# Refefer/Dampr

Hardware: AMD Instinct MI355X
Metric: tfidf_rows_per_sec (higher is better)
Workload: dtype int64-exact; 1 GPU; model=tfidf-docfreq, corpus_mb_per_gpu=10240, vocab=100000, global_batch=111848106, seq_len=96, parallelism=dp1

## Files before the change

dampr_amd/gpu/tfidf.py:

```python
import os

import torch

from ..ops import native
from .relational import _pow2_at_least

MODE_NEWLINE = 0
MODE_TOKEN_START = 1


def chunk_bounds(text, chunk_bytes):
    n = text.numel()
    bounds = [0]
    while bounds[-1] < n:
        e = min(bounds[-1] + chunk_bytes, n)
        if e < n:
            nl = torch.nonzero(text[e - 1:e + (1 << 16)] == ord("\n"))
            e = e + int(nl[0].item()) if nl.numel() else n
        bounds.append(e)
    return bounds


class TfidfEngine(object):
    def __init__(self, device, vocab_capacity=1 << 21):
        self.ext = native.require()
        self.device = torch.device(device)
        self.cap = _pow2_at_least(vocab_capacity)
        opts = dict(dtype=torch.int64, device=self.device)
        self.cnt_keys = torch.zeros(self.cap, **opts)
        self.cnt_vals = torch.zeros(self.cap, **opts)
        self.dict_keys = torch.zeros(self.cap, **opts)
        self.dict_vals = torch.zeros(self.cap, **opts)
        self.seen = None
        self._fb_seen = None
        self._err = None
        self._ablate = 0
        self.n_docs = 0

    def reset(self):
        self.cnt_keys.zero_()
        self.cnt_vals.zero_()
        self.dict_keys.zero_()
        self.dict_vals.zero_()
        self.n_docs = 0


    def positions(self, text, mode):
        counts = self.ext.mark_counts(text, mode).to(torch.int64)
        offsets = torch.cumsum(counts, 0) - counts
        total = int(offsets[-1].item() + counts[-1].item())
        out = torch.empty(total, dtype=torch.int32, device=self.device)
        self.ext.mark_positions(text, mode, offsets.to(torch.int32), out)
        return out, total


    def count_chunk(self, text, pos_base=0):
        assert text.numel() < (1 << 31), "chunk must be < 2 GiB"
        if self._fb_seen is None:
            self._fb_seen = torch.zeros(1 << 22, dtype=torch.int64,
                                        device=self.device)
            self._err = torch.zeros(4, dtype=torch.int32,
                                    device=self.device)
        else:
            self._fb_seen.zero_()
            self._err.zero_()
        snap = (self.cnt_keys.clone(), self.cnt_vals.clone(),
                self.dict_keys.clone(), self.dict_vals.clone())
        self.ext.tfidf_count_docs(text, self.cnt_keys, self.cnt_vals,
                                  self.dict_keys, self.dict_vals, pos_base,
                                  self._fb_seen, self._err, self._ablate)
        err, _, n_docs, _ = self._err.tolist()
        doc_base = self.n_docs
        self.n_docs += n_docs
        if err:
            (self.cnt_keys, self.cnt_vals,
             self.dict_keys, self.dict_vals) = snap
            nl, _ = self.positions(text, MODE_NEWLINE)
            self._count_chunk_general(text, nl, pos_base, doc_base)
        return n_docs

    def _count_chunk_general(self, text, nl, pos_base, doc_base):
        ts, n_tok = self.positions(text, MODE_TOKEN_START)
        seen_cap = _pow2_at_least(2 * max(n_tok, 1))
        if self.seen is None or self.seen.numel() < seen_cap:
            self.seen = torch.zeros(seen_cap, dtype=torch.int64,
                                    device=self.device)
        else:
            self.seen.zero_()
        self.ext.tfidf_count(text, nl, ts, self.seen, self.cnt_keys,
                             self.cnt_vals, self.dict_keys, self.dict_vals,
                             pos_base, doc_base)


    def extract(self):
        n_out = int((self.cnt_keys != 0).sum().item())
        out_k, out_v, _cur = self.ext.table_extract(
            self.cnt_keys, self.cnt_vals, n_out)
        order = torch.argsort(out_k)
        return out_k[order], out_v[order]


    def idf(self, df, total_docs):
        return self.ext.idf(df, float(total_docs))

    def _token_layout(self, keys):
        packed = self.ext.table_lookup(self.dict_keys, self.dict_vals, keys)
        lens = (packed & 0xFF).to(torch.int64)
        offsets = torch.cumsum(lens, 0) - lens
        total = int((offsets[-1] + lens[-1]).item()) if keys.numel() else 0
        return packed, lens, offsets, total

    def token_strings_dev(self, keys, text):
        packed, lens, offsets, total = self._token_layout(keys)
        blob = self.ext.gather_tokens(text, packed, offsets, total)
        return blob, lens

    def merge_exchanged(self, keys, df, blob, lens):
        self.cnt_keys.zero_()
        self.cnt_vals.zero_()
        self.dict_keys.zero_()
        self.dict_vals.zero_()
        self.ext.table_merge(keys, df, self.cnt_keys, self.cnt_vals)
        offsets = torch.cumsum(lens, 0) - lens
        packed = torch.bitwise_or(torch.bitwise_left_shift(offsets, 8),
                                  lens)
        self.ext.table_put(keys, packed, self.dict_keys, self.dict_vals)

    def token_strings(self, keys, text):
        blob, lens = self.token_strings_dev(keys, text)
        return blob.cpu().numpy(), lens.cpu().numpy()

    def sink_tsv_device(self, path, part_id, keys, df, idf, src_text):
        os.makedirs(path, exist_ok=True)
        packed, lens, tok_off, total_tok = self._token_layout(keys)
        sizes = self.ext.tsv_sizes(lens, df, idf)
        row_off = torch.cumsum(sizes, 0) - sizes
        total = int((row_off[-1] + sizes[-1]).item()) if keys.numel() else 0
        blob = self.ext.gather_tokens(src_text, packed, tok_off, total_tok)
        out = self.ext.tsv_format(blob, tok_off, lens, df, idf, row_off,
                                  total)
        with open(os.path.join(path, "part-{}".format(part_id)), "wb") as fh:
            fh.write(out.cpu().numpy().tobytes())


def run_tfidf(text_np, device="cuda:0", sink_path=None, chunk_bytes=None,
              engine=None):
    dev = torch.device(device)
    if isinstance(text_np, torch.Tensor):
        text = text_np.to(dev)
    else:
        text = torch.from_numpy(text_np).to(dev)
    eng = engine or TfidfEngine(dev)
    eng.reset()
    bounds = chunk_bounds(text, chunk_bytes or text.numel())
    for s, e in zip(bounds, bounds[1:]):
        eng.count_chunk(text[s:e].contiguous(), pos_base=s)
    keys, df = eng.extract()
    idf = eng.idf(df, eng.n_docs)
    blob, lens = eng.token_strings(keys, text)
    if sink_path:
        eng.sink_tsv_device(sink_path, 0, keys, df, idf, text)
    out = {}
    pos = 0
    b = blob.tobytes()
    df_np = df.cpu().numpy()
    idf_np = idf.cpu().numpy()
    for i in range(len(lens)):
        ln = int(lens[i])
        out[b[pos:pos + ln].decode("ascii")] = (int(df_np[i]),
                                                float(idf_np[i]))
        pos += ln
    return out
```

dampr_amd/ops/hip/dampr_kernels.hip:

```cpp
#include <hip/hip_runtime.h>
#include "host.h"

#include "common.h"

#define BLOCK 256
#define VBYTES 16
#define TILE (BLOCK * VBYTES)

#define MODE_NEWLINE 0
#define MODE_TOKEN_START 1

__device__ __forceinline__ bool mark_at(int mode, const u8* text,
                                        long i, long n) {
    u8 c = text[i];
    if (mode == MODE_NEWLINE) return c == '\n';
    if (!is_word(c)) return false;
    return i == 0 || !is_word(text[i - 1]);
}

__device__ __forceinline__ u32 nlmask32(u32 w) {
    u32 x = w ^ 0x0A0A0A0Au;
    return (x - 0x01010101u) & ~x & 0x80808080u;
}

__global__ void count_marks_kernel(const u8* __restrict__ text, long n,
                                   int mode, int iters,
                                   u32* __restrict__ counts) {
    long base = (long)blockIdx.x * iters * TILE;
    int tid = threadIdx.x;
    u32 local = 0;
    for (int it = 0; it < iters; ++it) {
        long off = base + (long)it * TILE + (long)tid * VBYTES;
        if (off >= n) break;
        if (off + VBYTES <= n) {
            uint4 v = *reinterpret_cast<const uint4*>(text + off);
            if (mode == MODE_NEWLINE) {
                local += __popc(nlmask32(v.x)) + __popc(nlmask32(v.y))
                       + __popc(nlmask32(v.z)) + __popc(nlmask32(v.w));
            } else {
                const u8* b = reinterpret_cast<const u8*>(&v);
                #pragma unroll
                for (int j = 0; j < VBYTES; ++j) {
                    bool prev_word = (j > 0)
                        ? is_word(b[j - 1])
                        : (off > 0 ? is_word(text[off - 1]) : false);
                    local += is_word(b[j]) && !prev_word;
                }
            }
        } else {
            for (long i = off; i < n; ++i)
                local += mark_at(mode, text, i, n);
        }
    }
    __shared__ u32 wsum[BLOCK / WAVE];
    for (int d = WAVE / 2; d > 0; d >>= 1)
        local += __shfl_down(local, d, WAVE);
    int lane = tid & (WAVE - 1), wid = tid / WAVE;
    if (lane == 0) wsum[wid] = local;
    __syncthreads();
    if (tid == 0) {
        u32 total = 0;
        for (int w = 0; w < BLOCK / WAVE; ++w) total += wsum[w];
        counts[blockIdx.x] = total;
    }
}

#define SCAN_MAX_ITERS 16

__device__ __forceinline__ u32 gather_marks(const u8* __restrict__ text,
                                            long n, int mode, long off,
                                            u8* rel) {
    u32 cnt = 0;
    if (off >= n) return 0;
    if (off + VBYTES <= n) {
        uint4 v = *reinterpret_cast<const uint4*>(text + off);
        if (mode == MODE_NEWLINE) {
            const u32 words[4] = {v.x, v.y, v.z, v.w};
            #pragma unroll
            for (int wi = 0; wi < 4; ++wi) {
                u32 m = nlmask32(words[wi]);
                while (m) {
                    int bit = __ffs(m) - 1;
                    rel[cnt++] = (u8)(wi * 4 + (bit >> 3));
                    m &= m - 1;
                }
            }
            return cnt;
        }
        const u8* b = reinterpret_cast<const u8*>(&v);
        #pragma unroll
        for (int j = 0; j < VBYTES; ++j) {
            u8 c = b[j];
            bool prev_word = (j > 0)
                ? is_word(b[j - 1])
                : (off > 0 ? is_word(text[off - 1]) : false);
            bool m = is_word(c) && !prev_word;
            if (m) rel[cnt++] = (u8)j;
        }
    } else {
        long lim = n - off;
        for (long j = 0; j < lim; ++j)
            if (mark_at(mode, text, off + j, n)) rel[cnt++] = (u8)j;
    }
    return cnt;
}

__global__ void write_marks_kernel(const u8* __restrict__ text, long n,
                                   int mode, int iters,
                                   const u32* __restrict__ block_offsets,
                                   u32* __restrict__ out) {
    long base = (long)blockIdx.x * iters * TILE;
    int tid = threadIdx.x;
    int lane = tid & (WAVE - 1), wid = tid / WAVE;
    __shared__ u32 wtile[BLOCK / WAVE][SCAN_MAX_ITERS];

    for (int it = 0; it < iters; ++it) {
        long off = base + (long)it * TILE + (long)tid * VBYTES;
        u8 rel[VBYTES];
        u32 cnt = gather_marks(text, n, mode, off, rel);
        u32 tot = cnt;
        for (int d = WAVE / 2; d > 0; d >>= 1)
            tot += __shfl_down(tot, d, WAVE);
        if (lane == 0) wtile[wid][it] = tot;
    }
    __syncthreads();

    u32 run = block_offsets[blockIdx.x];
    for (int it = 0; it < iters; ++it) {
        u32 wb = run;
        u32 tile_tot = 0;
        for (int w = 0; w < BLOCK / WAVE; ++w) {
            if (w < wid) wb += wtile[w][it];
            tile_tot += wtile[w][it];
        }
        long off = base + (long)it * TILE + (long)tid * VBYTES;
        u8 rel[VBYTES];
        u32 cnt = gather_marks(text, n, mode, off, rel);
        u32 scan = cnt;
        for (int d = 1; d < WAVE; d <<= 1) {
            u32 x = __shfl_up(scan, d, WAVE);
            if (lane >= d) scan += x;
        }
        u32 excl = wb + scan - cnt;
        for (u32 j = 0; j < cnt; ++j)
            out[excl + j] = (u32)(off + rel[j]);
        run += tile_tot;
    }
}

__global__ void tfidf_count_kernel(
        const u8* __restrict__ text, long n,
        const u32* __restrict__ nl_pos, long n_nl,
        const u32* __restrict__ tok_start, long n_tok,
        u64* __restrict__ seen_keys, u64 seen_mask,
        u64* __restrict__ cnt_keys, u64* __restrict__ cnt_vals,
        u64 cnt_mask,
        u64* __restrict__ dict_keys, u64* __restrict__ dict_vals,
        u64 dict_mask, u64 pos_base, u64 doc_base) {
    long stride = (long)gridDim.x * blockDim.x;
    for (long t = (long)blockIdx.x * blockDim.x + threadIdx.x; t < n_tok;
         t += stride) {
        u32 start = tok_start[t];
        long p = start;
        u64 h = 0;
        u32 j = 0;
        while (p < n) {
            u8 c = text[p];
            if (!is_word(c)) break;
            h = tokmix_step(h, j, lower_ascii(c));
            ++p;
            ++j;
        }
        u32 len = (u32)(p - start);
        h = tokmix_final(h, len);
        long lo = 0, hi = n_nl;
        while (lo < hi) {
            long mid = (lo + hi) >> 1;
            if (nl_pos[mid] < start) lo = mid + 1; else hi = mid;
        }
        u64 doc = (u64)lo + doc_base;
        u64 tok_key = h ? h : 1ULL;
        u64 sk = splitmix64(h ^ (doc * 0x9E3779B97F4A7C15ULL));
        if (!sk) sk = 1;
        u64 slot;
        if (table_insert_u64(seen_keys, seen_mask, sk, &slot)) {
            table_add_u64(cnt_keys, cnt_vals, cnt_mask, tok_key, 1ULL);
            if (table_insert_u64(dict_keys, dict_mask, tok_key, &slot))
                dict_vals[slot] = ((pos_base + (u64)start) << 8)
                                  | (u64)min(len, 255u);
        }
    }
}

#ifndef DOC_WAVES
#define DOC_WAVES 4
#endif
#ifndef STAGE_B
#define STAGE_B 2048
#endif
#define SEG_OVERLAP 272
#ifndef DOC_SET
#define DOC_SET 256
#endif
#ifndef FB_PROBE_CAP
#define FB_PROBE_CAP 512
#endif
#ifndef DOC_SPAN
#define DOC_SPAN 8192
#endif
#ifndef GROUP_BYTES
#define GROUP_BYTES 1024
#endif
#ifndef CCACHE
#define CCACHE 1024
#endif
#ifndef DOC_BPL
#define DOC_BPL 8
#endif
#define DOC_LENMIX_N 128
#define DOC_SALT_K 0x9E3779B97F4A7C15ULL
#define DOC_WIN (WAVE * DOC_BPL)
static_assert(DOC_BPL == 4 || DOC_BPL == 8, "lane word is b32 or b64");
static_assert(STAGE_B % 16 == 0, "stage edge on a lane boundary");
static_assert(DOC_SPAN % 16 == 0 && DOC_SPAN >= 16, "span on a 16 B edge");
static_assert(GROUP_BYTES == WAVE * 16 && GROUP_BYTES <= STAGE_B,
              "group search is one uint4 per lane of staged text");
#define GROUP_OPEN (1L << 62)

__device__ __forceinline__ u32 swar_ge(u32 x7, u32 k) {
    return x7 + (0x80u - k) * 0x01010101u;
}
__device__ __forceinline__ u32 swar_pack4(u32 m) {
    return (((m & 0x80808080u) >> 7) * 0x01020408u) >> 24;
}
__device__ __forceinline__ u32 wordbits4(u32 x) {
    const u32 x7 = x & 0x7F7F7F7Fu;
    const u32 y7 = x7 | 0x20202020u;
    const u32 m = (swar_ge(y7, 'a') ^ swar_ge(y7, 'z' + 1))
                | (swar_ge(x7, '0') ^ swar_ge(x7, '9' + 1))
                | (swar_ge(x7, '_') ^ swar_ge(x7, '_' + 1));
    return swar_pack4(m & ~x);
}
__device__ __forceinline__ u32 nlbits4(u32 x) {
    const u32 v = x ^ 0x0A0A0A0Au;
    return swar_pack4(~(((v & 0x7F7F7F7Fu) + 0x7F7F7F7Fu) | v));
}
__device__ __forceinline__ u32 nlbits16(const u8* p, long at, long from,
                                        long to) {
    const uint4 v = *reinterpret_cast<const uint4*>(p);
    const u32 m = nlbits4(v.x) | (nlbits4(v.y) << 4) | (nlbits4(v.z) << 8)
                | (nlbits4(v.w) << 12);
    const int lo = (int)min(max(from - at, 0L), 16L);
    const int hi = (int)min(max(to - at, 0L), 16L);
    return m & ((1u << hi) - 1u) & ~((1u << lo) - 1u);
}
__device__ __forceinline__ u32 nlbits_from(long at, long pos) {
    const int k = (int)min(max(pos - at, 0L), 16L);
    return ~((1u << k) - 1u);
}
__device__ __forceinline__ u64 low_bytes_mask(int k) {
    return k >= 8 ? ~0ULL : ((1ULL << (8 * k)) - 1ULL);
}

#define CC_PROBES 4
#define CC_HIT 0
#define CC_NEW 1
#define CC_MISS 2
#define EMIT_CNT 1u
#define EMIT_DICT 2u

__device__ __forceinline__ int block_cache_step(
        u64* __restrict__ cck, u32* __restrict__ ccv, u32 slot, u64 key,
        u64 cur) {
    if (cur == key) { atomicAdd(&ccv[slot], 1u); return CC_HIT; }
    if (cur == 0ULL) {
        const u64 prev = atomicCAS(&cck[slot], 0ULL, key);
        if (prev == 0ULL || prev == key) {
            atomicAdd(&ccv[slot], 1u);
            return prev == 0ULL ? CC_NEW : CC_HIT;
        }
    }
    return -1;
}

__device__ __forceinline__ int block_cache_add(
        u64* __restrict__ cck, u32* __restrict__ ccv, u64 key) {
    const u32 s0 = (u32)(key & (CCACHE - 1));
    u64 c[CC_PROBES];
    #pragma unroll
    for (int p = 0; p < CC_PROBES; ++p)
        c[p] = cck[(s0 + p) & (CCACHE - 1)];
    #pragma unroll
    for (int p = 0; p < CC_PROBES; ++p)
        asm volatile("" : "+v"(c[p]));
    int f = CC_PROBES;
    u64 cf = 0;
    #pragma unroll
    for (int p = CC_PROBES - 1; p >= 0; --p)
        if (c[p] == key || c[p] == 0ULL) { f = p; cf = c[p]; }
    if (f == CC_PROBES) return CC_MISS;
    u32 slot = (s0 + f) & (CCACHE - 1);
    int r = block_cache_step(cck, ccv, slot, key, cf);
    if (r >= 0) return r;
    for (int p = f + 1; p < CC_PROBES; ++p) {
        slot = (slot + 1) & (CCACHE - 1);
        r = block_cache_step(cck, ccv, slot, key, cck[slot]);
        if (r >= 0) return r;
    }
    return CC_MISS;
}

__device__ __forceinline__ int lds_set_insert(u64* set, u64 h) {
    u32 slot = (u32)(h & (DOC_SET - 1));
    for (int probe = 0; probe < DOC_SET; ++probe) {
        u64 prev = atomicCAS(&set[slot], 0ULL, h);
        if (prev == 0ULL) return 1;
        if (prev == h) return 0;
        slot = (slot + 1) & (DOC_SET - 1);
    }
    return -1;
}

__global__ void __launch_bounds__(DOC_WAVES * WAVE, 5)
tfidf_docs_kernel(const u8* __restrict__ text, long n,
                  u64* __restrict__ cnt_keys, u64* __restrict__ cnt_vals,
                  u64 cnt_mask,
                  u64* __restrict__ dict_keys, u64* __restrict__ dict_vals,
                  u64 dict_mask, u64 pos_base,
                  u64* __restrict__ fb_seen, u64 fb_mask,
                  u32* __restrict__ err_flag, u32 ablate) {
    __shared__ __align__(16) u8 stage[DOC_WAVES][STAGE_B + 16];
    __shared__ u64 dset[DOC_WAVES][DOC_SET];
    __shared__ u64 cck[CCACHE];
    __shared__ u32 ccv[CCACHE];
    __shared__ u64 toktab[256];
    __shared__ u64 lenmix[DOC_LENMIX_N];
    __shared__ u32 blk_docs;
    static_assert(sizeof(stage) + sizeof(dset) + sizeof(cck) + sizeof(ccv)
                  + sizeof(toktab) + sizeof(lenmix) + 8 <= 32768,
                  "block LDS allows 5 blocks per CU");
    const int wid = __builtin_amdgcn_readfirstlane(threadIdx.x / WAVE);
    const int lane = threadIdx.x % WAVE;
    const long gwave = (long)blockIdx.x * DOC_WAVES + wid;
    const long nwaves = (long)gridDim.x * DOC_WAVES;
    const long nspans = (n + DOC_SPAN - 1) / DOC_SPAN;
    u8* st = stage[wid];
    u64* set = dset[wid];
    u32 my_docs = 0;

    for (int i = threadIdx.x; i < CCACHE; i += blockDim.x) {
        cck[i] = 0;
        ccv[i] = 0;
    }
    for (int i = threadIdx.x; i < 256; i += blockDim.x)
        toktab[i] = is_word((u8)i) ? toktab_entry(lower_ascii((u8)i)) : 0ULL;
    for (int i = threadIdx.x; i < DOC_LENMIX_N; i += blockDim.x)
        lenmix[i] = splitmix64((u64)i);
    if (threadIdx.x == 0) blk_docs = 0;
    __syncthreads();

    auto finish_emit = [&](u64 key, u64 pk, u64 cw, u64 dw, u32 fl) {
        if ((fl & EMIT_DICT) && dw != key) {
            u64 slot;
            if (table_insert_u64(dict_keys, dict_mask, key, &slot))
                dict_vals[slot] = pk;
        }
        if (fl & EMIT_CNT) {
            if (cw == key) atomicAdd(&cnt_vals[key & cnt_mask], 1ULL);
            else table_add_u64(cnt_keys, cnt_vals, cnt_mask, key, 1ULL);
        }
    };

    for (long sp = gwave; sp < nspans; sp += nwaves) {
        const long a = sp * DOC_SPAN;
        const long b = a + DOC_SPAN;
        long win_lo = -1, win_hi = -1, aseg = 0;

        auto stage_at = [&](long seg) {
            aseg = seg & ~15L;
            const int stage_bytes =
                (int)min((long)(STAGE_B + 16), n - aseg);
            if (aseg + STAGE_B + 16 <= n) {
                #pragma unroll
                for (int i = 0; i < STAGE_B; i += WAVE * 16)
                    __builtin_amdgcn_global_load_lds(
                        (const u32*)(text + aseg + i + lane * 16),
                        (u32*)(st + i), 16, 0, 0);
                if (lane == 0)
                    __builtin_amdgcn_global_load_lds(
                        (const u32*)(text + aseg + STAGE_B),
                        (u32*)(st + STAGE_B), 16, 0, 0);
            } else {
                for (int i = lane * 16; i < stage_bytes; i += WAVE * 16) {
                    if (aseg + i + 16 <= n) {
                        *reinterpret_cast<uint4*>(st + i) =
                            *reinterpret_cast<const uint4*>(
                                text + aseg + i);
                    } else {
                        for (int j = i; j < stage_bytes; ++j)
                            st[j] = (aseg + j < n)
                                ? text[aseg + j] : (u8)0;
                    }
                }
            }
            __builtin_amdgcn_s_waitcnt(0x0070);
            asm volatile("" ::: "memory");
            __builtin_amdgcn_wave_barrier();
            win_lo = seg;
            win_hi = aseg + stage_bytes;
        };
        auto nl_lane16 = [&](long base, long from, long to) -> u32 {
            const long at = base + lane * 16;
            return at < to
                ? nlbits16(st + (int)(at - aseg), at, from, to) : 0u;
        };
        auto first_nl = [&](long from, long to) -> long {
            for (long base = from & ~15L; base < to; base += WAVE * 16) {
                const u32 m = nl_lane16(base, from, to);
                const u64 any = __ballot(m != 0);
                if (any) {
                    const int fl = __ffsll((unsigned long long)any) - 1;
                    const u32 mf = __builtin_amdgcn_readlane(m, fl);
                    return base + fl * 16 + (__ffs(mf) - 1);
                }
            }
            return -1;
        };

        long gs = 0;
        if (a > 0) {
            const long lim = min(b - 1, n);
            long p = -1;
            for (long pos = a - 1; pos < lim; ) {
                if (pos < win_lo || pos >= win_hi) stage_at(pos);
                const long to = min(win_hi, lim);
                p = first_nl(pos, to);
                if (p >= 0) break;
                pos = to;
            }
            if (p < 0) continue;
            gs = p + 1;
        }

        while (gs < n) {
            if (gs < win_lo || gs >= win_hi) stage_at(gs);
            const long gbase = gs & ~15L;
            long gend = GROUP_OPEN;
            for (int attempt = 0; attempt < 2; ++attempt) {
                const long to = min(gbase + (long)GROUP_BYTES, win_hi);
                const u32 m = nl_lane16(gbase, gs, to);
                const u32 mh = m & nlbits_from(gbase + lane * 16, b - 1);
                const u64 any = __ballot(m != 0);
                const u64 anyh = __ballot(mh != 0);
                if (anyh) {
                    const int fl = __ffsll((unsigned long long)anyh) - 1;
                    const u32 mf = __builtin_amdgcn_readlane(mh, fl);
                    gend = gbase + fl * 16 + (__ffs(mf) - 1);
                    break;
                }
                long last = -1;
                if (any) {
                    const int ll = 63 - __clzll((long long)any);
                    const u32 ml = __builtin_amdgcn_readlane(m, ll);
                    last = gbase + ll * 16 + (31 - __clz((int)ml));
                }
                if (to == n) {
                    gend = (last == n - 1) ? last : n;
                    break;
                }
                if (last >= 0) { gend = last; break; }
                if (to == gbase + (long)GROUP_BYTES) break;
                stage_at(gs);
            }

            for (int s = lane; s < DOC_SET; s += WAVE) set[s] = 0;
            u32 carry_word = 0;
            u32 carry_len = 0;
            u64 carry_g = 0;
            long carry_start = gs;
            u32 carry_lines = 0;

            auto emit_token = [&](u64 gh, u32 tl, long tbase, int trel,
                                  u32 drel) {
                if (ablate & 1) {
                    if (gh == 0xdeadbeefdeadbeefULL) err_flag[1] = 1;
                    return;
                }
                u64 lm;
                if (tl < DOC_LENMIX_N) lm = lenmix[tl];
                else lm = splitmix64((u64)tl);
                const u64 hh = gh ^ lm;
                const u64 key = hh ? hh : 1ULL;
                const long doc_id = gs + (long)drel;
                u64 dk = hh ^ ((u64)doc_id * DOC_SALT_K);
                if (!dk) dk = 1;
                int fresh = lds_set_insert(set, dk);
                if (fresh < 0) {
                    u64 sk = splitmix64(hh ^ ((u64)doc_id
                                              * 0x9E3779B97F4A7C15ULL));
                    if (!sk) sk = 1;
                    u64 slot = sk & fb_mask;
                    fresh = 0;
                    int probe = 0;
                    while (true) {
                        u64 prev = atomicCAS(&fb_seen[slot], 0ULL, sk);
                        if (prev == 0ULL) { fresh = 1; break; }
                        if (prev == sk) break;
                        slot = (slot + 1) & fb_mask;
                        if (++probe > FB_PROBE_CAP) {
                            atomicOr(err_flag, 1u);
                            break;
                        }
                    }
                }
                u32 fl = 0;
                if (fresh == 1 && !(ablate & 2)) {
                    const int cc = block_cache_add(cck, ccv, key);
                    if (cc == CC_MISS) fl |= EMIT_CNT;
                    if (!(ablate & 4) && cc != CC_HIT) fl |= EMIT_DICT;
                }
                const u64 pk = ((pos_base + (u64)(tbase + trel)) << 8)
                             | (u64)min(tl, 255u);
                u64 cw = 0, dw = 0;
                if (fl & EMIT_CNT) cw = cnt_keys[key & cnt_mask];
                if (fl & EMIT_DICT) dw = dict_keys[key & dict_mask];
                if (fl) finish_emit(key, pk, cw, dw, fl);
            };

            for (long seg = gs; seg < gend; ) {
                if (seg < win_lo || seg >= win_hi) stage_at(seg);
                if (gend == GROUP_OPEN) {
                    const long p = first_nl(seg, win_hi);
                    if (p >= 0) gend = p;
                    else if (win_hi == n) gend = n;
                }
                const long seg_end = min(gend, win_hi);
                const int soff = (int)(seg - aseg);
                const int soff_end = (int)(seg_end - aseg);
                const bool group_continues = seg_end < gend;
                for (int wb = soff & ~(DOC_BPL - 1); wb < soff_end;
                     wb += DOC_WIN) {
                    const int o = wb + lane * DOC_BPL;
                    const int keep_lo = min(max(soff - o, 0), DOC_BPL);
                    const int keep_hi = min(max(soff_end - o, 0), DOC_BPL);
                    u64 raw = 0;
                    if (keep_hi > 0) {
#if DOC_BPL == 8
                        raw = *reinterpret_cast<const u64*>(st + o);
#else
                        raw = *reinterpret_cast<const u32*>(st + o);
#endif
                    }
                    raw &= low_bytes_mask(keep_hi) & ~low_bytes_mask(keep_lo);
                    u32 W = wordbits4((u32)raw);
                    u32 NLb = nlbits4((u32)raw);
#if DOC_BPL == 8
                    W |= wordbits4((u32)(raw >> 32)) << 4;
                    NLb |= nlbits4((u32)(raw >> 32)) << 4;
#endif
                    u64 P[DOC_BPL];
                    u64 acc = 0, pz = 0;
                    u64 T[DOC_BPL];
                    #pragma unroll
                    for (int j = 0; j < DOC_BPL; ++j)
                        T[j] = toktab[(u32)(raw >> (8 * j)) & 0xFFu];
                    #pragma unroll
                    for (int j = 0; j < DOC_BPL; ++j)
                        asm volatile("" : "+v"(T[j]));
                    #pragma unroll
                    for (int j = 0; j < DOC_BPL; ++j) {
                        acc ^= rotl64(T[j], (u32)j);
                        pz = ((W >> j) & 1u) ? pz : acc;
                        P[j] = acc;
                    }
                    const bool first_w = W & 1u;
                    const bool last_w = (W >> (DOC_BPL - 1)) & 1u;
                    const u64 fw = __ballot(first_w);
                    const u64 lw = __ballot(last_w);
                    if (carry_word && !(fw & 1ULL)) {
                        if (lane == 0)
                            emit_token(carry_g, carry_len, carry_start,
                                       0, carry_lines);
                        carry_word = 0;
                        carry_len = 0;
                        carry_g = 0;
                    }
                    const int span = soff_end - wb;
                    const int e = span >= DOC_WIN ? WAVE - 1
                                                  : (span - 1) / DOC_BPL;
                    const bool hold = (e == WAVE - 1) || group_continues;
                    u64 nf = fw;
                    if (hold && e < WAVE - 1) nf |= 1ULL << (e + 1);
                    const bool next_first = (lane == WAVE - 1)
                        ? true : (bool)((nf >> (lane + 1)) & 1ULL);
                    const bool cont_in = first_w
                        && (lane == 0 ? carry_word != 0
                                      : (bool)((lw >> (lane - 1)) & 1ULL));
                    u32 E = W & ~((W >> 1)
                                  | ((u32)next_first << (DOC_BPL - 1)));

                    const u32 zb = ~W & ((1u << DOC_BPL) - 1u);
                    const int ts = zb ? 32 - __clz(zb) : 0;
                    u64 tg = 0;
                    u32 tlen = 0;
                    bool closed = true;
                    if (last_w) {
                        tg = rotl64(acc ^ pz, (u32)(64 - ts));
                        tlen = (u32)(DOC_BPL - ts);
                        closed = !(ts == 0 && cont_in);
                    }
                    for (int d = 1; d < WAVE; d <<= 1) {
                        if (!__ballot(!closed && lane >= d)) break;
                        const u64 ag = __shfl_up(tg, d, WAVE);
                        const u32 al = __shfl_up(tlen, d, WAVE);
                        const int ac = __shfl_up((int)closed, d, WAVE);
                        if (!closed && lane >= d) {
                            tg = ag ^ rotl64(tg, al);
                            tlen += al;
                            closed = ac;
                        }
                    }
                    if (!closed) {
                        tg = carry_g ^ rotl64(tg, carry_len);
                        tlen += carry_len;
                    }
                    u64 pg = __shfl_up(tg, 1, WAVE);
                    u32 plen = __shfl_up(tlen, 1, WAVE);
                    if (lane == 0) { pg = carry_g; plen = carry_len; }

                    const u32 nlc = __popc(NLb);
                    u32 nl_before = carry_lines;
                    for (u32 k = 1; ; ++k) {
                        const u64 b = __ballot(nlc >= k);
                        if (!b) break;
                        nl_before = __builtin_amdgcn_mbcnt_hi(
                            (u32)(b >> 32),
                            __builtin_amdgcn_mbcnt_lo((u32)b, nl_before));
                        carry_lines += (u32)__popcll(b);
                    }

                    if (((lw >> e) & 1ULL) && hold) {
                        carry_word = 1;
                        carry_g = __shfl(tg, e, WAVE);
                        carry_len = (u32)__shfl((int)tlen, e, WAVE);
                        carry_start = aseg + wb + (long)(e + 1) * DOC_BPL
                                      - (long)carry_len;
                    } else {
                        carry_word = 0;
                        carry_len = 0;
                        carry_g = 0;
                    }

                    u64 pprev = 0;
                    while (__ballot(E != 0)) {
                        if (E) {
                            const int j = __ffs(E) - 1;
                            E &= E - 1;
                            u64 pj = P[0];
                            #pragma unroll
                            for (int i = 1; i < DOC_BPL; ++i)
                                pj = (j == i) ? P[i] : pj;
                            const u32 zj = zb & ((1u << j) - 1u);
                            const int s = zj ? 32 - __clz(zj) : 0;
                            u64 g = rotl64(pj ^ pprev, (u32)(64 - s));
                            pprev = pj;
                            u32 len = (u32)(j - s + 1);
                            if (s == 0 && cont_in) {
                                g = pg ^ rotl64(g, plen);
                                len += plen;
                            }
                            emit_token(g, len, aseg,
                                       o + j + 1 - (int)len,
                                       nl_before
                                       + __popc(NLb & ((1u << j) - 1u)));
                        }
                    }
                }
                __builtin_amdgcn_wave_barrier();
                seg = seg_end;
            }
            if (carry_word) {
                if (lane == 0)
                    emit_token(carry_g, carry_len, carry_start, 0,
                               carry_lines);
            }
            my_docs += carry_lines + 1;
            if (gend >= b - 1) break;
            gs = gend + 1;
        }
    }
    if (lane == 0 && my_docs) atomicAdd(&blk_docs, my_docs);

    __syncthreads();
    if (threadIdx.x == 0 && blk_docs) atomicAdd(&err_flag[2], blk_docs);
    for (int i = threadIdx.x; i < CCACHE; i += blockDim.x)
        if (cck[i])
            table_add_u64(cnt_keys, cnt_vals, cnt_mask, cck[i],
                          (u64)ccv[i]);
}

__global__ void table_merge_kernel(const u64* __restrict__ in_keys,
                                   const long* __restrict__ in_vals,
                                   long n, u64* __restrict__ keys,
                                   u64* __restrict__ vals, u64 mask) {
    long stride = (long)gridDim.x * blockDim.x;
    for (long i = (long)blockIdx.x * blockDim.x + threadIdx.x; i < n;
         i += stride) {
        u64 k = in_keys[i];
        if (k) table_add_u64(keys, vals, mask, k, (u64)in_vals[i]);
    }
}

__global__ void table_put_kernel(const u64* __restrict__ in_keys,
                                 const u64* __restrict__ in_vals, long n,
                                 u64* __restrict__ keys,
                                 u64* __restrict__ vals, u64 mask) {
    long stride = (long)gridDim.x * blockDim.x;
    for (long i = (long)blockIdx.x * blockDim.x + threadIdx.x; i < n;
         i += stride) {
        u64 k = in_keys[i];
        if (!k) continue;
        u64 slot;
        if (table_insert_u64(keys, mask, k, &slot))
            vals[slot] = in_vals[i];
    }
}

__global__ void table_extract_kernel(const u64* __restrict__ keys,
                                     const u64* __restrict__ vals,
                                     long cap, u64* __restrict__ out_k,
                                     long* __restrict__ out_v,
                                     u64* __restrict__ cursor) {
    long stride = (long)gridDim.x * blockDim.x;
    for (long i = (long)blockIdx.x * blockDim.x + threadIdx.x; i < cap;
         i += stride) {
        u64 k = keys[i];
        if (k) {
            u64 j = atomicAdd(cursor, 1ULL);
            out_k[j] = k;
            out_v[j] = (long)vals[i];
        }
    }
}

__global__ void table_lookup_kernel(const u64* __restrict__ keys,
                                    const u64* __restrict__ vals, u64 mask,
                                    const u64* __restrict__ query, long n,
                                    u64* __restrict__ out) {
    long stride = (long)gridDim.x * blockDim.x;
    for (long i = (long)blockIdx.x * blockDim.x + threadIdx.x; i < n;
         i += stride) {
        u64 k = query[i];
        u64 slot = k & mask;
        u64 r = 0;
        while (true) {
            u64 cur = keys[slot];
            if (cur == k) { r = vals[slot]; break; }
            if (cur == 0) break;
            slot = (slot + 1) & mask;
        }
        out[i] = r;
    }
}

__global__ void idf_kernel(const long* __restrict__ df, long n,
                           double total, double* __restrict__ out) {
    long stride = (long)gridDim.x * blockDim.x;
    for (long i = (long)blockIdx.x * blockDim.x + threadIdx.x; i < n;
         i += stride)
        out[i] = log(1.0 + total / (double)df[i]);
}

__global__ void gather_tokens_kernel(const u8* __restrict__ text,
                                     const u64* __restrict__ packed, long n,
                                     const long* __restrict__ offsets,
                                     u8* __restrict__ out) {
    long stride = (long)gridDim.x * blockDim.x;
    for (long i = (long)blockIdx.x * blockDim.x + threadIdx.x; i < n;
         i += stride) {
        u64 pk = packed[i];
        u32 pos = (u32)(pk >> 8);
        u32 len = (u32)(pk & 0xFF);
        long o = offsets[i];
        for (u32 j = 0; j < len; ++j)
            out[o + j] = lower_ascii(text[pos + j]);
    }
}


__device__ __forceinline__ int dec_digits_u64(u64 v) {
    int d = 1;
    while (v >= 10) { v /= 10; ++d; }
    return d;
}

__device__ __forceinline__ void fmt_idf_parts(double x, u64* int_part,
                                              u64* frac_part) {
    double scaled = x * 1e9 + 0.5;
    u64 v = (u64)scaled;
    *int_part = v / 1000000000ULL;
    *frac_part = v % 1000000000ULL;
}

__global__ void tsv_sizes_kernel(const long* __restrict__ lens,
                                 const long* __restrict__ df,
                                 const double* __restrict__ idf, long n,
                                 long* __restrict__ sizes) {
    long stride = (long)gridDim.x * blockDim.x;
    for (long i = (long)blockIdx.x * blockDim.x + threadIdx.x; i < n;
         i += stride) {
        u64 ip, fp;
        fmt_idf_parts(idf[i], &ip, &fp);
        sizes[i] = lens[i] + 1 + dec_digits_u64((u64)df[i]) + 1
                 + dec_digits_u64(ip) + 1 + 9 + 1;
    }
}

__device__ __forceinline__ u8* write_u64_dec(u8* p, u64 v, int width) {
    for (int j = width - 1; j >= 0; --j) { p[j] = '0' + (v % 10); v /= 10; }
    return p + width;
}

__global__ void tsv_format_kernel(const u8* __restrict__ blob,
                                  const long* __restrict__ tok_off,
                                  const long* __restrict__ lens,
                                  const long* __restrict__ df,
                                  const double* __restrict__ idf,
                                  const long* __restrict__ row_off, long n,
                                  u8* __restrict__ out) {
    long stride = (long)gridDim.x * blockDim.x;
    for (long i = (long)blockIdx.x * blockDim.x + threadIdx.x; i < n;
         i += stride) {
        u8* p = out + row_off[i];
        const u8* t = blob + tok_off[i];
        for (long j = 0; j < lens[i]; ++j) *p++ = t[j];
        *p++ = '\t';
        u64 d = (u64)df[i];
        p = write_u64_dec(p, d, dec_digits_u64(d));
        *p++ = '\t';
        u64 ip, fp;
        fmt_idf_parts(idf[i], &ip, &fp);
        p = write_u64_dec(p, ip, dec_digits_u64(ip));
        *p++ = '.';
        p = write_u64_dec(p, fp, 9);
        *p++ = '\n';
    }
}


namespace {

inline int grid_for(long work, int block = BLOCK, int cap = 4096) {
    long g = (work + block - 1) / block;
    return (int)std::min<long>(std::max<long>(g, 1), cap);
}

void check_u8(const torch::Tensor& t) {
    TORCH_CHECK(t.is_cuda() && t.dtype() == torch::kUInt8 &&
                t.is_contiguous(), "expected contiguous u8 device tensor");
}

constexpr int SCAN_ITERS = 8;

}

torch::Tensor mark_counts(torch::Tensor text, long mode) {
    check_u8(text);
    long n = text.numel();
    long span = (long)SCAN_ITERS * TILE;
    long nblocks = (n + span - 1) / span;
    auto counts = torch::empty({std::max(nblocks, 1L)},
        torch::TensorOptions().dtype(torch::kUInt32).device(text.device()));
    if (n == 0) { counts.zero_(); return counts; }
    hipLaunchKernelGGL(count_marks_kernel, dim3((u32)nblocks), dim3(BLOCK),
                       0, cur_stream(), text.data_ptr<u8>(), n, (int)mode,
                       SCAN_ITERS, (u32*)counts.data_ptr());
    return counts;
}

void mark_positions(torch::Tensor text, long mode,
                    torch::Tensor block_offsets, torch::Tensor out) {
    check_u8(text);
    long n = text.numel();
    if (n == 0 || out.numel() == 0) return;
    long span = (long)SCAN_ITERS * TILE;
    long nblocks = (n + span - 1) / span;
    hipLaunchKernelGGL(write_marks_kernel, dim3((u32)nblocks), dim3(BLOCK),
                       0, cur_stream(), text.data_ptr<u8>(), n, (int)mode,
                       SCAN_ITERS, (u32*)block_offsets.data_ptr(),
                       (u32*)out.data_ptr());
}

void tfidf_count(torch::Tensor text, torch::Tensor nl_pos,
                 torch::Tensor tok_start, torch::Tensor seen_keys,
                 torch::Tensor cnt_keys, torch::Tensor cnt_vals,
                 torch::Tensor dict_keys, torch::Tensor dict_vals,
                 long pos_base, long doc_base) {
    check_u8(text);
    long n_tok = tok_start.numel();
    if (n_tok == 0) return;
    hipLaunchKernelGGL(tfidf_count_kernel,
        dim3(grid_for(n_tok)), dim3(BLOCK), 0, cur_stream(),
        text.data_ptr<u8>(), text.numel(),
        (const u32*)nl_pos.data_ptr(), nl_pos.numel(),
        (const u32*)tok_start.data_ptr(), n_tok,
        (u64*)seen_keys.data_ptr(), (u64)(seen_keys.numel() - 1),
        (u64*)cnt_keys.data_ptr(), (u64*)cnt_vals.data_ptr(),
        (u64)(cnt_keys.numel() - 1),
        (u64*)dict_keys.data_ptr(), (u64*)dict_vals.data_ptr(),
        (u64)(dict_keys.numel() - 1), (u64)pos_base, (u64)doc_base);
}

void tfidf_count_docs(torch::Tensor text, torch::Tensor cnt_keys,
                      torch::Tensor cnt_vals, torch::Tensor dict_keys,
                      torch::Tensor dict_vals, long pos_base,
                      torch::Tensor fb_seen, torch::Tensor meta,
                      long ablate) {
    check_u8(text);
    TORCH_CHECK(meta.is_cuda() && meta.is_contiguous()
                && meta.scalar_type() == torch::kInt32
                && meta.numel() >= 3, "meta must be device int32[>=3]");
    TORCH_CHECK(text.numel() < (1L << 31), "chunk must be < 2 GiB");
    const long n = text.numel();
    if (n == 0) return;
    long waves_needed = (n + DOC_SPAN - 1) / DOC_SPAN;
    long blocks = std::min<long>((waves_needed + DOC_WAVES - 1) / DOC_WAVES,
                                 8192);
    hipLaunchKernelGGL(tfidf_docs_kernel, dim3((u32)blocks),
        dim3(DOC_WAVES * WAVE), 0, cur_stream(),
        text.data_ptr<u8>(), n,
        (u64*)cnt_keys.data_ptr(), (u64*)cnt_vals.data_ptr(),
        (u64)(cnt_keys.numel() - 1),
        (u64*)dict_keys.data_ptr(), (u64*)dict_vals.data_ptr(),
        (u64)(dict_keys.numel() - 1), (u64)pos_base,
        (u64*)fb_seen.data_ptr(), (u64)(fb_seen.numel() - 1),
        (u32*)meta.data_ptr(), (u32)ablate);
}

long tfidf_span_bytes() { return DOC_SPAN; }

void table_merge(torch::Tensor in_keys, torch::Tensor in_vals,
                 torch::Tensor keys, torch::Tensor vals) {
    long n = in_keys.numel();
    if (n == 0) return;
    hipLaunchKernelGGL(table_merge_kernel, dim3(grid_for(n)), dim3(BLOCK),
        0, cur_stream(), (const u64*)in_keys.data_ptr(),
        in_vals.data_ptr<long>(), n, (u64*)keys.data_ptr(),
        (u64*)vals.data_ptr(), (u64)(keys.numel() - 1));
}

void table_put(torch::Tensor in_keys, torch::Tensor in_vals,
               torch::Tensor keys, torch::Tensor vals) {
    long n = in_keys.numel();
    if (n == 0) return;
    hipLaunchKernelGGL(table_put_kernel, dim3(grid_for(n)), dim3(BLOCK),
        0, cur_stream(), (const u64*)in_keys.data_ptr(),
        (const u64*)in_vals.data_ptr(), n, (u64*)keys.data_ptr(),
        (u64*)vals.data_ptr(), (u64)(keys.numel() - 1));
}

std::vector<torch::Tensor> table_extract(torch::Tensor keys,
                                         torch::Tensor vals, long n_out) {
    auto dev = keys.device();
    auto out_k = torch::empty({n_out},
        torch::TensorOptions().dtype(torch::kInt64).device(dev));
    auto out_v = torch::empty({n_out},
        torch::TensorOptions().dtype(torch::kInt64).device(dev));
    auto cursor = torch::zeros({1},
        torch::TensorOptions().dtype(torch::kInt64).device(dev));
    long cap = keys.numel();
    if (cap > 0 && n_out > 0)
        hipLaunchKernelGGL(table_extract_kernel, dim3(grid_for(cap)),
            dim3(BLOCK), 0, cur_stream(), (const u64*)keys.data_ptr(),
            (const u64*)vals.data_ptr(), cap, (u64*)out_k.data_ptr(),
            out_v.data_ptr<long>(), (u64*)cursor.data_ptr());
    return {out_k, out_v, cursor};
}

torch::Tensor table_lookup(torch::Tensor keys, torch::Tensor vals,
                           torch::Tensor query) {
    long n = query.numel();
    auto out = torch::zeros({n},
        torch::TensorOptions().dtype(torch::kInt64).device(query.device()));
    if (n > 0)
        hipLaunchKernelGGL(table_lookup_kernel, dim3(grid_for(n)),
            dim3(BLOCK), 0, cur_stream(), (const u64*)keys.data_ptr(),
            (const u64*)vals.data_ptr(), (u64)(keys.numel() - 1),
            (const u64*)query.data_ptr(), n, (u64*)out.data_ptr());
    return out;
}

torch::Tensor idf(torch::Tensor df, double total) {
    long n = df.numel();
    auto out = torch::empty({n},
        torch::TensorOptions().dtype(torch::kFloat64).device(df.device()));
    if (n > 0)
        hipLaunchKernelGGL(idf_kernel, dim3(grid_for(n)), dim3(BLOCK), 0,
            cur_stream(), df.data_ptr<long>(), n, total,
            out.data_ptr<double>());
    return out;
}

torch::Tensor gather_tokens(torch::Tensor text, torch::Tensor packed,
                            torch::Tensor offsets, long total_bytes) {
    check_u8(text);
    long n = packed.numel();
    auto out = torch::empty({std::max(total_bytes, 1L)},
        torch::TensorOptions().dtype(torch::kUInt8).device(text.device()));
    if (n > 0)
        hipLaunchKernelGGL(gather_tokens_kernel, dim3(grid_for(n)),
            dim3(BLOCK), 0, cur_stream(), text.data_ptr<u8>(),
            (const u64*)packed.data_ptr(), n, offsets.data_ptr<long>(),
            out.data_ptr<u8>());
    return out;
}

torch::Tensor tsv_sizes(torch::Tensor lens, torch::Tensor df,
                        torch::Tensor idf) {
    long n = lens.numel();
    auto out = torch::empty({std::max(n, 1L)},
        torch::TensorOptions().dtype(torch::kInt64).device(lens.device()));
    if (n > 0)
        hipLaunchKernelGGL(tsv_sizes_kernel, dim3(grid_for(n)), dim3(BLOCK),
            0, cur_stream(), lens.data_ptr<long>(), df.data_ptr<long>(),
            idf.data_ptr<double>(), n, out.data_ptr<long>());
    return out;
}

torch::Tensor tsv_format(torch::Tensor blob, torch::Tensor tok_off,
                         torch::Tensor lens, torch::Tensor df,
                         torch::Tensor idf, torch::Tensor row_off,
                         long total_bytes) {
    long n = lens.numel();
    auto out = torch::empty({std::max(total_bytes, 1L)},
        torch::TensorOptions().dtype(torch::kUInt8).device(blob.device()));
    if (n > 0)
        hipLaunchKernelGGL(tsv_format_kernel, dim3(grid_for(n)),
            dim3(BLOCK), 0, cur_stream(), blob.data_ptr<u8>(),
            tok_off.data_ptr<long>(), lens.data_ptr<long>(),
            df.data_ptr<long>(), idf.data_ptr<double>(),
            row_off.data_ptr<long>(), n, out.data_ptr<u8>());
    return out;
}

torch::Tensor rs_hist(torch::Tensor keys, long shift, long nblocks);
torch::Tensor rs_digit_fold(torch::Tensor keys);
void rs_scatter(torch::Tensor keys, torch::Tensor payload,
                torch::Tensor scanned, long shift, long nblocks,
                torch::Tensor out_k, torch::Tensor out_p);
void seg_reduce(torch::Tensor seg, torch::Tensor vals, torch::Tensor out,
                long op);
void hj_build(torch::Tensor keys_r, torch::Tensor t_keys,
              torch::Tensor t_head, torch::Tensor next);
torch::Tensor hj_count(torch::Tensor keys_l, torch::Tensor t_keys,
                       torch::Tensor t_head, torch::Tensor next,
                       long left_outer);
long rs_span();
torch::Tensor seg_count(torch::Tensor keys);
void seg_reduce_fused(torch::Tensor keys, torch::Tensor vals,
                      torch::Tensor tile_base, long op,
                      torch::Tensor out_keys, torch::Tensor out_vals);
void mp_merge(torch::Tensor ka, torch::Tensor pa, torch::Tensor kb,
              torch::Tensor pb, long bias_signed, torch::Tensor out_k,
              torch::Tensor out_p);
void varlen_gather(torch::Tensor blob, torch::Tensor src_off,
                   torch::Tensor lens, torch::Tensor new_offs,
                   torch::Tensor out);
std::vector<torch::Tensor> hj_emit(torch::Tensor keys_l,
                                   torch::Tensor t_keys,
                                   torch::Tensor t_head,
                                   torch::Tensor next,
                                   torch::Tensor offsets, long total,
                                   long left_outer, long track_matched,
                                   long nr);

void sv_hash64(torch::Tensor blob, torch::Tensor offs, uint64_t mask,
               torch::Tensor out);
void sv_adjacent_eq(torch::Tensor blob, torch::Tensor offs,
                    torch::Tensor sorted_hash, torch::Tensor perm,
                    torch::Tensor heads, torch::Tensor n_mismatch);
void sv_lex_key(torch::Tensor blob, torch::Tensor offs, torch::Tensor rows,
                long d, torch::Tensor out);
void sv_lex_refine(torch::Tensor grp_sorted, torch::Tensor key_sorted,
                   torch::Tensor heads, torch::Tensor open);

long filter_tile();
torch::Tensor filter_count(torch::Tensor keys, torch::Tensor vals,
                           std::vector<int64_t> prog);
void filter_scatter(torch::Tensor keys, torch::Tensor vals,
                    std::vector<int64_t> prog, torch::Tensor block_off,
                    torch::Tensor out_k, torch::Tensor out_v);

long sv_filter_tile();
long sv_filter_max_const();
torch::Tensor sv_filter_count(c10::optional<torch::Tensor> keys,
                              torch::Tensor blob, torch::Tensor offs,
                              std::vector<int64_t> prog,
                              torch::Tensor consts);
void sv_filter_scatter(torch::Tensor keys, torch::Tensor blob,
                       torch::Tensor offs, std::vector<int64_t> prog,
                       torch::Tensor consts, torch::Tensor block_off,
                       torch::Tensor out_k, torch::Tensor out_src,
                       torch::Tensor out_len);

PYBIND11_MODULE(TORCH_EXTENSION_NAME, m) {
    m.def("filter_tile", &filter_tile,
          "rows per filter block (dampr_filter.hip FILTER_TILE)");
    m.def("filter_count", &filter_count,
          "survivors of a clause program per tile (compaction, pass 1)");
    m.def("filter_scatter", &filter_scatter,
          "stable scatter of the surviving rows (compaction, pass 2)");
    m.def("sv_filter_tile", &sv_filter_tile,
          "rows per string-filter block (dampr_strfilter.hip SVF_TILE)");
    m.def("sv_filter_max_const", &sv_filter_max_const,
          "longest string constant of a clause, in bytes");
    m.def("sv_filter_count", &sv_filter_count,
          "survivors of a key/string clause program per tile (pass 1)");
    m.def("sv_filter_scatter", &sv_filter_scatter,
          "surviving rows' keys, arena offsets and lengths, stable (pass 2)");
    m.def("rs_hist", &rs_hist, "radix pass histogram (bin-major)");
    m.def("rs_digit_fold", &rs_digit_fold,
          "AND/OR fold over keys (constant-digit skip detection)");
    m.def("rs_scatter", &rs_scatter, "stable radix scatter pass");
    m.def("seg_reduce", &seg_reduce,
          "segmented reduce over sorted runs (op 0=sum,1=min,2=max)");
    m.def("hj_build", &hj_build, "hash-join build (chained)");
    m.def("varlen_gather", &varlen_gather,
          "row gather for byte-arena value columns");
    m.def("sv_hash64", &sv_hash64,
          "strmix64(row) & mask per row of a byte-arena column");
    m.def("sv_adjacent_eq", &sv_adjacent_eq,
          "segment heads over hash-sorted rows, byte-verified");
    m.def("sv_lex_key", &sv_lex_key,
          "u64 order key of the 7-byte window d of the given rows");
    m.def("sv_lex_refine", &sv_lex_refine,
          "class heads and still-undecided rows over (group, key) order");
    m.def("rs_span", &rs_span,
          "elements per radix block (dampr_sort.hip RS_SPAN)");
    m.def("seg_count", &seg_count,
          "segment-start counts per tile (fused group-by, pass 1)");
    m.def("seg_reduce_fused", &seg_reduce_fused,
          "fused boundary-derive + segmented reduce over sorted keys");
    m.def("mp_merge", &mp_merge,
          "stable merge-path 2-way merge of sorted (key, payload) runs");
    m.def("hj_count", &hj_count, "hash-join probe match counts");
    m.def("hj_emit", &hj_emit, "hash-join emit (l,r) row-index pairs");
    m.def("tsv_sizes", &tsv_sizes, "per-row TSV byte sizes");
    m.def("tsv_format", &tsv_format, "format token/df/idf rows as TSV");
    m.def("mark_counts", &mark_counts,
          "per-block counts of marks (mode 0=newline, 1=token start)");
    m.def("mark_positions", &mark_positions,
          "write ascending mark positions given exclusive block offsets");
    m.def("tfidf_count", &tfidf_count,
          "tokenize+hash+per-doc-dedupe+df-count in one pass");
    m.def("tfidf_count_docs", &tfidf_count_docs,
          "span-per-wave tokenize+dedupe+count (fast path); counts docs");
    m.def("tfidf_span_bytes", &tfidf_span_bytes,
          "text bytes a wave of tfidf_count_docs owns per visit");
    m.def("table_merge", &table_merge, "add (k,v) pairs into a hash table");
    m.def("table_put", &table_put,
          "insert (k,v) pairs if absent (first writer wins)");
    m.def("table_extract", &table_extract,
          "compact non-empty table slots to (keys, vals, count)");
    m.def("table_lookup", &table_lookup, "probe table for query keys");
    m.def("idf", &idf, "idf = log(1 + total/df)");
    m.def("gather_tokens", &gather_tokens,
          "materialize token byte strings from dict entries");
}
```

Baseline: 4.512 billion rows/s.

## Snapshot only count values and compact table extraction with wave ballots

The per-chunk rollback snapshot now clones only the count-value table instead of all four hash tables, which removes three full-table device copies per chunk. This assumes the fast kernel leaves keys and dictionary entries safe to keep on the error path. The table extraction kernel is replaced with a tiled stream compaction: each wave ballots its non-empty slots, the block takes one atomic reservation for its total, and lanes write at computed offsets instead of doing one global atomic per key. The fallback seen-buffer size also becomes a constructor parameter.

```diff
diff --git a/dampr_amd/gpu/tfidf.py b/dampr_amd/gpu/tfidf.py
--- a/dampr_amd/gpu/tfidf.py
+++ b/dampr_amd/gpu/tfidf.py
@@ -22,7 +22,8 @@
 
 
 class TfidfEngine(object):
-    def __init__(self, device, vocab_capacity=1 << 21):
+    def __init__(self, device, vocab_capacity=1 << 21,
+                 fallback_seen_capacity=1 << 22):
         self.ext = native.require()
         self.device = torch.device(device)
         self.cap = _pow2_at_least(vocab_capacity)
@@ -34,6 +35,7 @@
         self.seen = None
         self._fb_seen = None
         self._err = None
+        self._fb_cap = _pow2_at_least(fallback_seen_capacity)
         self._ablate = 0
         self.n_docs = 0
 
@@ -57,15 +59,14 @@
     def count_chunk(self, text, pos_base=0):
         assert text.numel() < (1 << 31), "chunk must be < 2 GiB"
         if self._fb_seen is None:
-            self._fb_seen = torch.zeros(1 << 22, dtype=torch.int64,
+            self._fb_seen = torch.zeros(self._fb_cap, dtype=torch.int64,
                                         device=self.device)
             self._err = torch.zeros(4, dtype=torch.int32,
                                     device=self.device)
         else:
             self._fb_seen.zero_()
             self._err.zero_()
-        snap = (self.cnt_keys.clone(), self.cnt_vals.clone(),
-                self.dict_keys.clone(), self.dict_vals.clone())
+        snap_vals = self.cnt_vals.clone()
         self.ext.tfidf_count_docs(text, self.cnt_keys, self.cnt_vals,
                                   self.dict_keys, self.dict_vals, pos_base,
                                   self._fb_seen, self._err, self._ablate)
@@ -73,8 +74,7 @@
         doc_base = self.n_docs
         self.n_docs += n_docs
         if err:
-            (self.cnt_keys, self.cnt_vals,
-             self.dict_keys, self.dict_vals) = snap
+            self.cnt_vals = snap_vals
             nl, _ = self.positions(text, MODE_NEWLINE)
             self._count_chunk_general(text, nl, pos_base, doc_base)
         return n_docs
diff --git a/dampr_amd/ops/hip/dampr_kernels.hip b/dampr_amd/ops/hip/dampr_kernels.hip
--- a/dampr_amd/ops/hip/dampr_kernels.hip
+++ b/dampr_amd/ops/hip/dampr_kernels.hip
@@ -2,6 +2,7 @@
 #include "host.h"
 
 #include "common.h"
+#include "compact.h"
 
 #define BLOCK 256
 #define VBYTES 16
@@ -726,21 +727,44 @@
     }
 }
 
-__global__ void table_extract_kernel(const u64* __restrict__ keys,
-                                     const u64* __restrict__ vals,
-                                     long cap, u64* __restrict__ out_k,
-                                     long* __restrict__ out_v,
-                                     u64* __restrict__ cursor) {
-    long stride = (long)gridDim.x * blockDim.x;
-    for (long i = (long)blockIdx.x * blockDim.x + threadIdx.x; i < cap;
-         i += stride) {
-        u64 k = keys[i];
-        if (k) {
-            u64 j = atomicAdd(cursor, 1ULL);
-            out_k[j] = k;
-            out_v[j] = (long)vals[i];
-        }
-    }
+__global__ void __launch_bounds__(COMPACT_BLOCK)
+table_extract_kernel(const u64* __restrict__ keys,
+                     const u64* __restrict__ vals, long cap,
+                     u64* __restrict__ out_k, long* __restrict__ out_v,
+                     long n_out, u64* __restrict__ cursor) {
+    __shared__ u64 tile_base;
+    const long base = compact_first_row();
+    u64 k[COMPACT_STRIPS];
+    u64 ballots[COMPACT_STRIPS];
+    int cnt = 0;
+#pragma unroll
+    for (int s = 0; s < COMPACT_STRIPS; ++s) {
+        const long slot = base + (long)s * WAVE;
+        k[s] = slot < cap ? keys[slot] : 0ULL;
+    }
+#pragma unroll
+    for (int s = 0; s < COMPACT_STRIPS; ++s) {
+        ballots[s] = __ballot(k[s] != 0ULL);
+        cnt += __popcll(ballots[s]);
+    }
+    const int* wave_cnt = compact_wave_counts(cnt);
+    if (threadIdx.x == 0) {
+        int total = 0;
+#pragma unroll
+        for (int w = 0; w < COMPACT_WAVES; ++w) total += wave_cnt[w];
+        tile_base = total ? atomicAdd(cursor, (u64)total) : 0ULL;
+    }
+    __syncthreads();
+    long pos = (long)tile_base;
+#pragma unroll
+    for (int w = 0; w < COMPACT_WAVES; ++w)
+        if (w < compact_wave()) pos += wave_cnt[w];
+#pragma unroll
+    for (int s = 0; s < COMPACT_STRIPS; ++s)
+        pos = compact_emit(ballots[s], pos, n_out, [&](long o) {
+            out_k[o] = k[s];
+            out_v[o] = (long)vals[base + (long)s * WAVE];
+        });
 }
 
 __global__ void table_lookup_kernel(const u64* __restrict__ keys,
@@ -969,11 +993,16 @@
     auto cursor = torch::zeros({1},
         torch::TensorOptions().dtype(torch::kInt64).device(dev));
     long cap = keys.numel();
-    if (cap > 0 && n_out > 0)
-        hipLaunchKernelGGL(table_extract_kernel, dim3(grid_for(cap)),
-            dim3(BLOCK), 0, cur_stream(), (const u64*)keys.data_ptr(),
-            (const u64*)vals.data_ptr(), cap, (u64*)out_k.data_ptr(),
-            out_v.data_ptr<long>(), (u64*)cursor.data_ptr());
+    TORCH_CHECK(n_out >= 0 && vals.numel() >= cap,
+                "table_extract: n_out >= 0 and a value per slot");
+    if (cap > 0) {
+        const long tiles = (cap + COMPACT_TILE - 1) / COMPACT_TILE;
+        hipLaunchKernelGGL(table_extract_kernel, dim3((u32)tiles),
+            dim3(COMPACT_BLOCK), 0, cur_stream(),
+            (const u64*)keys.data_ptr(), (const u64*)vals.data_ptr(), cap,
+            (u64*)out_k.data_ptr(), out_v.data_ptr<long>(), n_out,
+            (u64*)cursor.data_ptr());
+    }
     return {out_k, out_v, cursor};
 }
 
```

Result: faster. 4.630 billion rows/s, median of 6 (+2.6%).
